# sourmash-bio/sourmash

Measured on AMD Instinct MI355X. Metric: Gbase/s sketched (k=31, scaled=1000), higher is better.
Workload: dtype u64; 1 GPU; C2: sketch synthetic random DNA resident in HBM as ASCII, per GPU 1000 records of 10000000 bases (10000000000 bases, 10000001000 bytes with their separators), k=31 scaled=1000 seed=42; one step = k-mer kernel + radix sort + unique; records_per_gpu=1000, record_len=10000000, bases_per_gpu=10000000000, bytes_per_gpu=10000001000, ksize=31, scaled=1000, unique_hashes_rank0=9998668, unique_hashes_job=9998668, collectives=none (the exchange runs with --full)

## Files before the change

### sourmash_amd/csrc/kmer_core.hpp

```cpp
#pragma once
#include "murmur3.hpp"
#include <utility>

namespace smg {

SMG_HD uint32_t perm_b32(uint32_t hi, uint32_t lo, uint32_t sel) {
#if defined(__HIP_DEVICE_COMPILE__)
    return __builtin_amdgcn_perm(hi, lo, sel);
#else
    const uint64_t v = ((uint64_t)hi << 32) | lo;
    uint32_t r = 0;
    for (int i = 0; i < 4; ++i) {
        const uint32_t s = (sel >> (8 * i)) & 0xff;
        uint32_t b;
        if (s < 8) b = (uint32_t)(v >> (8 * s)) & 0xff;
        else if (s == 0x0c) b = 0;
        else b = 0xff;
        r |= b << (8 * i);
    }
    return r;
#endif
}

SMG_HD uint32_t alignbyte_b32(uint32_t hi, uint32_t lo, uint32_t n) {
#if defined(__HIP_DEVICE_COMPILE__)
    return __builtin_amdgcn_alignbyte(hi, lo, n);
#else
    return (uint32_t)((((uint64_t)hi << 32) | lo) >> (8 * n));
#endif
}

SMG_HD bool any_lane(bool p) {
#if defined(__HIP_DEVICE_COMPILE__)
    return __builtin_amdgcn_ballot_w64(p) != 0ull;
#else
    return p;
#endif
}

SMG_HD uint32_t bitselect(uint32_t mask, uint32_t b, uint32_t c) {
#if defined(__HIP_DEVICE_COMPILE__)
    return __builtin_amdgcn_bitop3_b32(mask, b, c, 0xCA);
#else
    return (mask & b) | (~mask & c);
#endif
}

SMG_HD uint32_t opaque(uint32_t x) {
#if defined(__HIP_DEVICE_COMPILE__)
    asm volatile("" : "+v"(x));
#endif
    return x;
}

SMG_HD uint32_t bswap32(uint32_t x) { return perm_b32(0u, x, 0x00010203u); }

constexpr uint32_t LUT_SELF = 'A' | ('C' << 8) | ('T' << 16) | ((uint32_t)'G' << 24);
constexpr uint32_t LUT_COMP = 'T' | ('G' << 8) | ('A' << 16) | ((uint32_t)'C' << 24);

template <int K, int P>
struct LaneGeom {
    static constexpr int NBYTES = P + K - 1;
    static constexpr int NW = (NBYTES + 3) / 4;
    static constexpr int NWK = (K + 3) / 4;
    static constexpr int NCH = (K + 7) / 8;
    static constexpr uint32_t LAST_MASK = (K % 4) ? ((1u << (8 * (K % 4))) - 1u) : 0xffffffffu;
};

constexpr uint32_t rev_sel(int a) {
    return (uint32_t)(a + 3) | ((uint32_t)(a + 2) << 8) | ((uint32_t)(a + 1) << 16) | ((uint32_t)a << 24);
}
constexpr uint32_t rev_sel_partial(int a, int nb) {
    uint32_t s = 0;
    for (int i = 0; i < 4; ++i) {
        const uint32_t b = (i < nb) ? (uint32_t)(a + nb - 1 - i) : 0x0cu;
        s |= b << (8 * i);
    }
    return s;
}

template <int K, int P, int O>
struct PosOps {
    using G = LaneGeom<K, P>;

    template <int D>
    static SMG_HD uint32_t fwd(const uint32_t* U) {
        constexpr int q = (O >> 2) + D, a = O & 3;
        uint32_t v;
        if constexpr (a == 0) v = U[q];
        else if constexpr (q + 1 < G::NW) v = alignbyte_b32(U[q + 1], U[q], a);
        else v = U[q] >> (8 * a);
        if constexpr (D == G::NWK - 1) v &= G::LAST_MASK;
        return v;
    }

    template <int D>
    static SMG_HD uint32_t rev(const uint32_t* C) {
        constexpr int nb = (K - 4 * D) >= 4 ? 4 : (K - 4 * D);
        constexpr int s = O + K - 4 * D - nb;
        constexpr int q = s >> 2, a = s & 3;
        constexpr uint32_t sel = (nb == 4) ? rev_sel(a) : rev_sel_partial(a, nb);
        if constexpr (q + 1 < G::NW) return perm_b32(C[q + 1], C[q], sel);
        else return perm_b32(0u, C[q], sel);
    }

    template <int CH>
    static SMG_HD uint64_t be_chunk(const uint32_t* W) {
        uint64_t v = (uint64_t)bswap32(W[2 * CH]) << 32;
        if constexpr (2 * CH + 1 < G::NWK) v |= bswap32(W[2 * CH + 1]);
        return v;
    }

    template <int CH>
    static SMG_HD uint64_t be_chunk_opaque(const uint32_t* W) {
        uint64_t v = (uint64_t)bswap32(opaque(W[2 * CH])) << 32;
        if constexpr (2 * CH + 1 < G::NWK) v |= bswap32(opaque(W[2 * CH + 1]));
        return v;
    }

    template <int CH>
    static SMG_HD void tie_break(const uint32_t* F, const uint32_t* R, bool& tie, bool& gt) {
        if constexpr (CH < G::NCH) {
            const uint64_t bf = be_chunk_opaque<CH>(F), br = be_chunk_opaque<CH>(R);
            gt = gt || (tie && bf > br);
            tie = tie && (bf == br);
            tie_break<CH + 1>(F, R, tie, gt);
        }
    }

    template <int... D>
    static SMG_HD void build(const uint32_t* U, const uint32_t* C, uint32_t* F, uint32_t* R,
                             std::integer_sequence<int, D...>) {
        ((F[D] = fwd<D>(U)), ...);
        ((R[D] = rev<D>(C)), ...);
    }

    template <bool PLAIN = false>
    static SMG_HD Mmh3Open hash_open(const uint32_t* U, const uint32_t* C, uint64_t seed) {
        uint32_t F[G::NWK], R[G::NWK];
        build(U, C, F, R, std::make_integer_sequence<int, G::NWK>{});
        const uint64_t bf = be_chunk<0>(F), br = be_chunk<0>(R);
        bool gt = bf > br;
        bool tie = bf == br;
        if (G::NCH > 1 && any_lane(tie)) tie_break<1>(F, R, tie, gt);
        uint32_t W[G::NWK];
        const uint32_t m = gt ? 0xffffffffu : 0u;
#pragma unroll
        for (int d = 0; d < G::NWK; ++d) W[d] = bitselect(m, R[d], F[d]);
        return mmh3_open_words<K, PLAIN>(W, seed);
    }
};

SMG_HD uint32_t nonzero_bytes4(uint32_t x) {
    uint32_t t = x | (x >> 4);
    t |= t >> 2;
    t |= t >> 1;
    t &= 0x01010101u;
    return (t * 0x01020408u) >> 24 & 0xfu;
}

SMG_HD uint32_t early_limit(uint64_t thr) {
    const uint32_t thr_hi = (uint32_t)(thr >> 32);
    return thr_hi >= 0xfffffffdu ? 0xffffffffu : thr_hi + 2u;
}
SMG_HD bool early_may_keep(Mmh3Open open, uint32_t lim) { return (uint32_t)(mmh3_close_hi_sum(open) + 1u) <= lim; }

template <int K, int P, bool EARLY, bool PLAIN, bool STAGED, class Emit, int... O>
SMG_HD void process_window(const uint32_t* raw, const uint32_t* comp, bool dirty, uint64_t seed, uint64_t thr, Emit&& emit,
                           std::integer_sequence<int, O...>) {
    using G = LaneGeom<K, P>;
    const uint32_t lim = early_limit(thr);
    uint32_t Ubuf[STAGED ? 1 : G::NW], Cbuf[STAGED ? 1 : G::NW];
    const uint32_t* U = STAGED ? raw : Ubuf;
    const uint32_t* C = STAGED ? comp : Cbuf;
    uint32_t anybad = 0;
    if constexpr (!STAGED) {
#pragma unroll
        for (int i = 0; i < G::NW; ++i) {
            const uint32_t u = raw[i] & 0xdfdfdfdfu;
            const uint32_t code = (u >> 1) & 0x03030303u;
            Ubuf[i] = u;
            Cbuf[i] = perm_b32(0u, LUT_COMP, code);
            uint32_t bad = perm_b32(0u, LUT_SELF, code) ^ u;
            if (i == G::NW - 1 && (G::NBYTES % 4) != 0)
                bad &= (1u << (8 * (G::NBYTES % 4))) - 1u;
            anybad |= bad;
        }
    }
    uint64_t badlo = 0, badhi = 0, badtop = 0;
    if (!STAGED || dirty) {
        if constexpr (STAGED) {
#pragma unroll
            for (int i = 0; i < G::NW; ++i) {
                const uint32_t u = U[i];
                uint32_t bad = perm_b32(0u, LUT_SELF, (u >> 1) & 0x03030303u) ^ u;
                if (i == G::NW - 1 && (G::NBYTES % 4) != 0)
                    bad &= (1u << (8 * (G::NBYTES % 4))) - 1u;
                anybad |= bad;
            }
        }
        if (anybad != 0) {
#pragma unroll
            for (int i = 0; i < G::NW; ++i) {
                const uint32_t u = U[i];
                const uint32_t code = (u >> 1) & 0x03030303u;
                uint32_t bad = perm_b32(0u, LUT_SELF, code) ^ u;
                if (i == G::NW - 1 && (G::NBYTES % 4) != 0) bad &= (1u << (8 * (G::NBYTES % 4))) - 1u;
                const uint64_t nib = nonzero_bytes4(bad);
                if (4 * i < 64) badlo |= nib << (4 * i);
                else if (4 * i < 128) badhi |= nib << (4 * i - 64);
                else badtop |= nib << (4 * i - 128);
            }
        }
    }
    static_assert(G::NBYTES <= 192 && K <= 128 && P <= 64, "window too long for the 192-bit validity mask");
    (
        [&] {
            const Mmh3Open open = PosOps<K, P, O>::template hash_open<PLAIN>(U, C, seed);
            if constexpr (EARLY) {
                if (!any_lane(early_may_keep(open, lim))) return;
            }
            const uint64_t h = mmh3_close<PLAIN>(open);
            bool ok = (h - 1) < thr;
            if (anybad != 0) {
                uint64_t lo, hi;
                if constexpr (O == 0) { lo = badlo; hi = badhi; }
                else { lo = (badlo >> O) | (badhi << (64 - O)); hi = (badhi >> O) | (badtop << (64 - O)); }
                const uint64_t mlo = K >= 64 ? ~0ull : ((1ull << K) - 1);
                const uint64_t mhi = K >= 128 ? ~0ull : K > 64 ? ((1ull << (K - 64)) - 1) : 0;
                if ((lo & mlo) | (hi & mhi)) ok = false;
            }
            if (ok) emit(O, h);
        }(),
        ...);
}

template <int K, int P, bool EARLY = true, bool PLAIN = false, class Emit>
SMG_HD void process_lane(const uint32_t* raw, uint64_t seed, uint64_t thr, Emit&& emit) {
    process_window<K, P, EARLY, PLAIN, false>(raw, nullptr, false, seed, thr, static_cast<Emit&&>(emit),
                                              std::make_integer_sequence<int, P>{});
}
template <int K, int P, bool EARLY = true, bool PLAIN = false, class Emit>
SMG_HD void process_lane_staged(const uint32_t* U, const uint32_t* C, bool dirty, uint64_t seed, uint64_t thr, Emit&& emit) {
    process_window<K, P, EARLY, PLAIN, true>(U, C, dirty, seed, thr, static_cast<Emit&&>(emit), std::make_integer_sequence<int, P>{});
}


template <int K, int P, int BLOCK>
struct TileGeom {
    using G = LaneGeom<K, P>;
    static constexpr int TILE = BLOCK * P;
    static constexpr int LANE_RD = ((G::NW + 3) / 4) * 4;
    static constexpr int IN_DW = (BLOCK - 1) * (P / 4) + LANE_RD;
    static constexpr int IN_CHUNKS = (IN_DW + 3) / 4;
};

SMG_HD void load_chunk(const uint8_t* seq, uint64_t off, uint64_t len, uint32_t skip, uint32_t* w) {
    w[0] = w[1] = w[2] = w[3] = 0;
    if (off + 16 <= len) {
#if defined(__HIP_DEVICE_COMPILE__)
        const uint4 v = *reinterpret_cast<const uint4*>(seq + off);
        w[0] = v.x; w[1] = v.y; w[2] = v.z; w[3] = v.w;
#else
        for (int b = 0; b < 16; ++b) w[b >> 2] |= (uint32_t)seq[off + b] << (8 * (b & 3));
#endif
    } else if (off < len) {
        for (uint64_t b = off; b < len; ++b) w[(b - off) >> 2] |= (uint32_t)seq[b] << (8 * ((b - off) & 3));
    }
    if (off == 0 && skip) {
        for (uint32_t b = 0; b < skip; ++b) w[b >> 2] &= ~(0xffu << (8 * (b & 3)));
    }
}

SMG_HD uint32_t stage_chunk(uint32_t* w, uint32_t* c) {
    uint32_t anybad = 0;
#pragma unroll
    for (int j = 0; j < 4; ++j) {
        const uint32_t u = w[j] & 0xdfdfdfdfu;
        const uint32_t code = (u >> 1) & 0x03030303u;
        w[j] = u;
        c[j] = perm_b32(0u, LUT_COMP, code);
        anybad |= perm_b32(0u, LUT_SELF, code) ^ u;
    }
    return anybad;
}

SMG_HD void store_chunk(uint32_t* dst, const uint32_t* w) {
#if defined(__HIP_DEVICE_COMPILE__)
    *reinterpret_cast<uint4*>(dst) = make_uint4(w[0], w[1], w[2], w[3]);
#else
    dst[0] = w[0]; dst[1] = w[1]; dst[2] = w[2]; dst[3] = w[3];
#endif
}

template <int IN_CHUNKS, bool STAGED, int BLOCK>
SMG_HD void stage_tile(const uint8_t* seq, uint64_t base, uint64_t len, uint32_t skip, uint32_t* s_in, uint32_t* s_comp,
                       unsigned int* s_dirty) {
#if defined(__HIP_DEVICE_COMPILE__)
    const int first = threadIdx.x, step = BLOCK;
#else
    const int first = 0, step = 1;
#endif
    for (int c = first; c < IN_CHUNKS; c += step) {
        uint32_t w[4];
        load_chunk(seq, base + (uint64_t)c * 16, len, skip, w);
        if constexpr (STAGED) {
            uint32_t cw[4];
            if (stage_chunk(w, cw)) *s_dirty = 1;
            store_chunk(&s_comp[c * 4], cw);
        }
        store_chunk(&s_in[c * 4], w);
    }
}

template <int LANE_RD, int P>
SMG_HD void read_window(const uint32_t* s, int tid, uint32_t* out) {
    static_assert(P % 4 == 0 && LANE_RD % 4 == 0, "lane runs must start dword aligned");
    const uint32_t* p = &s[tid * (P / 4)];
#pragma unroll
    for (int i = 0; i < LANE_RD / 4; ++i) {
#if defined(__HIP_DEVICE_COMPILE__)
        if constexpr ((P / 4) % 4 == 0) {
            const uint4 v = reinterpret_cast<const uint4*>(p)[i];
            out[4 * i] = v.x; out[4 * i + 1] = v.y; out[4 * i + 2] = v.z; out[4 * i + 3] = v.w;
            continue;
        }
#endif
        out[4 * i] = p[4 * i]; out[4 * i + 1] = p[4 * i + 1]; out[4 * i + 2] = p[4 * i + 2]; out[4 * i + 3] = p[4 * i + 3];
    }
}

#if defined(__HIPCC__)
template <int CAP, int BLOCK, int NV = 1>
struct LdsSink {
    uint64_t* s_val[NV];
    unsigned int* s_cnt;
    unsigned long long* s_base;
    uint64_t* out[NV];
    unsigned long long* out_count;
    uint64_t out_cap;

    template <class... V>
    __device__ __forceinline__ void append(V... v) const {
        static_assert(sizeof...(V) == NV, "one value per array");
        const uint64_t e[NV] = {(uint64_t)v...};
        const unsigned int idx = atomicAdd(s_cnt, 1u);
        if (idx < (unsigned)CAP) {
#pragma unroll
            for (int j = 0; j < NV; ++j) s_val[j][idx] = e[j];
        } else {
            const unsigned long long g = atomicAdd(out_count, 1ull);
            if (g < out_cap) {
#pragma unroll
                for (int j = 0; j < NV; ++j) out[j][g] = e[j];
            }
        }
    }
    __device__ __forceinline__ void flush(unsigned int at_least) const {
        const unsigned int cnt = *s_cnt;
        if (cnt < at_least) return;
        const unsigned int n = cnt < (unsigned)CAP ? cnt : (unsigned)CAP;
        if (threadIdx.x == 0) *s_base = atomicAdd(out_count, (unsigned long long)n);
        __syncthreads();
        const unsigned long long b = *s_base;
        for (unsigned int i = threadIdx.x; i < n; i += BLOCK) {
            if (b + i < out_cap) {
#pragma unroll
                for (int j = 0; j < NV; ++j) out[j][b + i] = s_val[j][i];
            }
        }
        __syncthreads();
        if (threadIdx.x == 0) *s_cnt = 0;
    }
};
#endif

}
```

### sourmash_amd/csrc/sketch_kernel.hpp

```cpp
#pragma once
#include <hip/hip_runtime.h>
#include <stdint.h>
#include <utility>
#include "kmer_core.hpp"
#include "tile_launch.hpp"

namespace smg {

constexpr int SK_BLOCK = 256;
constexpr int SK_FAST_MAX_K = 88;
constexpr int SK_OUT_CAP = 2048;

constexpr bool sk_plain_mul(int k, bool dense) {
    if (dense) return k == 1 || k == 5 || k == 8 || k == 25 || k == 28 || k == 81 || k == 82 || k == 84;
    return k == 50 || k == 51;
}
constexpr bool sk_staged(int k) { return k > 11 && k != 18 && k != 20 && k != 30; }

template <int K, int P, bool DENSE>
__global__ __launch_bounds__(SK_BLOCK) void sketch_dna_kernel(
    const uint8_t* __restrict__ seq, uint64_t len, uint64_t seed, uint64_t thr,
    uint64_t* __restrict__ out, unsigned long long* __restrict__ out_count, uint64_t out_cap,
    uint64_t n_tiles, uint32_t skip) {
    using T = TileGeom<K, P, SK_BLOCK>;
    constexpr int TILE = T::TILE, LANE_RD = T::LANE_RD, IN_CHUNKS = T::IN_CHUNKS;
    constexpr bool STAGED = !DENSE && sk_staged(K);

    __shared__ __attribute__((aligned(16))) uint32_t s_in[IN_CHUNKS * 4];
    __shared__ __attribute__((aligned(16))) uint32_t s_comp[STAGED ? IN_CHUNKS * 4 : 4];
    __shared__ unsigned int s_dirty;
    __shared__ uint64_t s_out[SK_OUT_CAP];
    __shared__ unsigned int s_cnt;
    __shared__ unsigned long long s_base;
    const LdsSink<SK_OUT_CAP, SK_BLOCK> sink{{s_out}, &s_cnt, &s_base, {out}, out_count, out_cap};

    const int tid = threadIdx.x;
    if (tid == 0) s_cnt = 0;

    for (uint64_t tile = blockIdx.x; tile < n_tiles; tile += gridDim.x) {
        const uint64_t base = tile * (uint64_t)TILE;
        if constexpr (STAGED) {
            if (tid == 0) s_dirty = 0;
        }
        __syncthreads();
        if constexpr (STAGED) {
            stage_tile<IN_CHUNKS, true, SK_BLOCK>(seq, base, len, skip, s_in, s_comp, &s_dirty);
        } else {
            for (int c = tid; c < IN_CHUNKS; c += SK_BLOCK) {
                const uint64_t off = base + (uint64_t)c * 16;
                uint4 v = make_uint4(0, 0, 0, 0);
                if (off + 16 <= len) {
                    v = *reinterpret_cast<const uint4*>(seq + off);
                } else if (off < len) {
                    uint32_t w[4] = {0, 0, 0, 0};
                    for (uint64_t b = off; b < len; ++b) w[(b - off) >> 2] |= (uint32_t)seq[b] << (8 * ((b - off) & 3));
                    v = make_uint4(w[0], w[1], w[2], w[3]);
                }
                if (off == 0 && skip) {
                    uint32_t w[4] = {v.x, v.y, v.z, v.w};
                    for (uint32_t b = 0; b < skip; ++b) w[b >> 2] &= ~(0xffu << (8 * (b & 3)));
                    v = make_uint4(w[0], w[1], w[2], w[3]);
                }
                *reinterpret_cast<uint4*>(&s_in[c * 4]) = v;
            }
        }
        __syncthreads();
        uint32_t raw[LANE_RD];
        read_window<LANE_RD, P>(s_in, tid, raw);
        auto emit = [&](int o, uint64_t h) {
            if constexpr (DENSE) {
                const uint64_t pos = base + (uint64_t)tid * P + (uint64_t)o - skip;
                if (pos < out_cap) out[pos] = h;
            } else {
                sink.append(h);
            }
        };
        if constexpr (STAGED) {
            static_assert(!STAGED || P == 16, "the staged form reads whole 16-byte groups");
            uint32_t comp[LANE_RD];
            read_window<LANE_RD, P>(s_comp, tid, comp);
            const bool dirty = __builtin_amdgcn_readfirstlane(s_dirty) != 0;
            process_lane_staged<K, P, true, sk_plain_mul(K, false)>(raw, comp, dirty, seed, thr, emit);
        } else {
            process_lane<K, P, !DENSE, sk_plain_mul(K, DENSE)>(raw, seed, thr, emit);
        }
        if constexpr (DENSE) continue;
        __syncthreads();
        sink.flush(SK_OUT_CAP / 2);
    }
    if constexpr (DENSE) return;
    __syncthreads();
    sink.flush(1);
}

typedef hipError_t (*sketch_launch_fn)(const uint8_t*, uint64_t, uint64_t, uint64_t, uint64_t*, unsigned long long*, uint64_t, hipStream_t);
template <bool DENSE>
struct SketchLaunch {
    using fn = sketch_launch_fn;
    static constexpr int KMAX = SK_FAST_MAX_K;
    template <int K>
    static hipError_t launch(const uint8_t* d_seq, uint64_t len, uint64_t seed, uint64_t thr, uint64_t* d_out,
                             unsigned long long* d_count, uint64_t cap, hipStream_t stream) {
        const TileSpan t = align_to_tiles(d_seq, len, (uint64_t)SK_BLOCK * 16);
        if (t.n_tiles == 0) return hipSuccess;
        hipLaunchKernelGGL((sketch_dna_kernel<K, 16, DENSE>), dim3(sk_grid(t.n_tiles)), dim3(SK_BLOCK), 0, stream, t.seq, t.len, seed,
                           thr, d_out, d_count, cap, t.n_tiles, t.skip);
        return hipGetLastError();
    }
};

}
```

### sourmash_amd/csrc/tile_launch.hpp

```cpp
#pragma once
#include <hip/hip_runtime.h>
#include <stdint.h>
#include <utility>

namespace smg {

struct TileSpan {
    const uint8_t* seq;
    uint64_t len;
    uint32_t skip;
    uint64_t n_tiles;
};
inline TileSpan align_to_tiles(const uint8_t* d_seq, uint64_t len, uint64_t tile_positions) {
    const uint32_t skip = (uint32_t)((uintptr_t)d_seq & 15);
    return {d_seq - skip, len + skip, skip, (len + skip + tile_positions - 1) / tile_positions};
}

inline unsigned sk_grid(uint64_t n_tiles) {
    const uint64_t max_blocks = 256ull * 8;
    return (unsigned)(n_tiles < max_blocks ? n_tiles : max_blocks);
}
inline unsigned lds_grid(uint64_t n_tiles, bool lds) {
    uint64_t g = sk_grid(n_tiles);
    if (lds && g > 256 && g > n_tiles / 8) g = n_tiles / 8 > 256 ? n_tiles / 8 : 256;
    return (unsigned)g;
}

template <auto Kernel>
hipError_t allow_dynamic_lds(size_t bytes, size_t most) {
    if (bytes <= 48 * 1024) return hipSuccess;
    static const hipError_t allowed = hipFuncSetAttribute((const void*)Kernel, hipFuncAttributeMaxDynamicSharedMemorySize, (int)most);
    return allowed;
}

constexpr int K_PART = 16;

template <class F, int K0, int... KS>
typename F::fn k_launcher_from(uint32_t k, std::integer_sequence<int, KS...>) {
    static const typename F::fn table[] = {&F::template launch<K0 + KS + 1>...};
    return table[k - K0 - 1];
}
template <class F, int PART>
typename F::fn part_launcher(uint32_t k);
template <class F>
typename F::fn launcher(uint32_t k) {
    static_assert(F::KMAX > 5 * K_PART && F::KMAX <= 6 * K_PART, "six parts");
    switch ((k - 1u) / (uint32_t)K_PART) {
    case 0: return part_launcher<F, 0>(k);
    case 1: return part_launcher<F, 1>(k);
    case 2: return part_launcher<F, 2>(k);
    case 3: return part_launcher<F, 3>(k);
    case 4: return part_launcher<F, 4>(k);
    default: return part_launcher<F, 5>(k);
    }
}
#define SMG_KMER_PART(F, PART)                                                                                                   \
    template <>                                                                                                                  \
    typename F::fn part_launcher<F, PART>(uint32_t k) {                                                                          \
        constexpr int K0 = K_PART * (PART), N = F::KMAX - K0 < K_PART ? F::KMAX - K0 : K_PART;                                   \
        return k_launcher_from<F, K0>(k, std::make_integer_sequence<int, N>());                                                  \
    }

}
```

Measured before the change: 334.1 Gbase/s.

## Stage multiple rounds per tile in LDS and enlarge sketch grid

For staged k>17, each workgroup now loads a tile covering up to three 4096-base windows into LDS with one pair of barriers and one sink flush, then loops over the rounds. This amortises synchronisation, halo reloads and flush overhead across more positions. The LDS output buffer is halved to fit and the grid per CU grows from 8 to 32. Rounds fall back to one when the expected hashes per tile might overflow the smaller sink.

```diff
diff --git a/sourmash_amd/csrc/kmer_core.hpp b/sourmash_amd/csrc/kmer_core.hpp
--- a/sourmash_amd/csrc/kmer_core.hpp
+++ b/sourmash_amd/csrc/kmer_core.hpp
@@ -246,14 +246,23 @@
 }
 
 
-template <int K, int P, int BLOCK>
+template <int K, int P, int BLOCK, int R = 1>
 struct TileGeom {
     using G = LaneGeom<K, P>;
-    static constexpr int TILE = BLOCK * P;
+    static constexpr int WINDOW = BLOCK * P;
+    static constexpr int TILE = R * WINDOW;
     static constexpr int LANE_RD = ((G::NW + 3) / 4) * 4;
-    static constexpr int IN_DW = (BLOCK - 1) * (P / 4) + LANE_RD;
-    static constexpr int IN_CHUNKS = (IN_DW + 3) / 4;
+    static constexpr int chunks(int rounds) { return ((rounds * BLOCK - 1) * (P / 4) + LANE_RD + 3) / 4; }
+    static constexpr int IN_DW = (R * BLOCK - 1) * (P / 4) + LANE_RD;
+    static constexpr int IN_CHUNKS = chunks(R);
 };
+
+SMG_HD uint32_t sk_tile_rounds(uint64_t thr, uint32_t r_max, uint32_t window, uint32_t cap) {
+    if (r_max <= 1) return 1;
+    const uint64_t positions = (uint64_t)r_max * window;
+    const uint64_t expected = (positions * (thr >> 32)) >> 32;
+    return expected + 1 > cap / 4 ? 1u : r_max;
+}
 
 SMG_HD void load_chunk(const uint8_t* seq, uint64_t off, uint64_t len, uint32_t skip, uint32_t* w) {
     w[0] = w[1] = w[2] = w[3] = 0;
@@ -295,13 +304,13 @@
 
 template <int IN_CHUNKS, bool STAGED, int BLOCK>
 SMG_HD void stage_tile(const uint8_t* seq, uint64_t base, uint64_t len, uint32_t skip, uint32_t* s_in, uint32_t* s_comp,
-                       unsigned int* s_dirty) {
+                       unsigned int* s_dirty, int n_chunks = IN_CHUNKS) {
 #if defined(__HIP_DEVICE_COMPILE__)
     const int first = threadIdx.x, step = BLOCK;
 #else
     const int first = 0, step = 1;
 #endif
-    for (int c = first; c < IN_CHUNKS; c += step) {
+    for (int c = first; c < n_chunks; c += step) {
         uint32_t w[4];
         load_chunk(seq, base + (uint64_t)c * 16, len, skip, w);
         if constexpr (STAGED) {
diff --git a/sourmash_amd/csrc/sketch_kernel.hpp b/sourmash_amd/csrc/sketch_kernel.hpp
--- a/sourmash_amd/csrc/sketch_kernel.hpp
+++ b/sourmash_amd/csrc/sketch_kernel.hpp
@@ -16,35 +16,52 @@
     return k == 50 || k == 51;
 }
 constexpr bool sk_staged(int k) { return k > 11 && k != 18 && k != 20 && k != 30; }
+#ifndef SMG_SK_R_MAX
+#define SMG_SK_R_MAX 3
+#endif
+constexpr int SK_R_MAX = SMG_SK_R_MAX;
+static_assert(SK_R_MAX >= 1 && SK_R_MAX <= 3, "four rounds do not fit four workgroups per CU");
+constexpr bool sk_one_round(int k) { return k <= 17; }
+constexpr int sk_rounds_max(int k, bool dense) { return !dense && sk_staged(k) && !sk_one_round(k) ? SK_R_MAX : 1; }
+constexpr int sk_out_cap(int r_max) { return r_max >= 3 ? SK_OUT_CAP / 2 : SK_OUT_CAP; }
+#ifdef SMG_SK_GRID_PER_CU
+constexpr unsigned sk_grid_per_cu(int) { return SMG_SK_GRID_PER_CU; }
+#else
+constexpr unsigned sk_grid_per_cu(int r_max) { return r_max > 1 ? 32 : 8; }
+#endif
 
 template <int K, int P, bool DENSE>
 __global__ __launch_bounds__(SK_BLOCK) void sketch_dna_kernel(
     const uint8_t* __restrict__ seq, uint64_t len, uint64_t seed, uint64_t thr,
     uint64_t* __restrict__ out, unsigned long long* __restrict__ out_count, uint64_t out_cap,
-    uint64_t n_tiles, uint32_t skip) {
-    using T = TileGeom<K, P, SK_BLOCK>;
-    constexpr int TILE = T::TILE, LANE_RD = T::LANE_RD, IN_CHUNKS = T::IN_CHUNKS;
+    uint64_t n_tiles, uint32_t skip, uint32_t rounds) {
+    constexpr int R_MAX = sk_rounds_max(K, DENSE), OUT_CAP = sk_out_cap(R_MAX);
+    using T = TileGeom<K, P, SK_BLOCK, R_MAX>;
+    constexpr int WINDOW = T::WINDOW, LANE_RD = T::LANE_RD, IN_CHUNKS = T::IN_CHUNKS;
     constexpr bool STAGED = !DENSE && sk_staged(K);
+    static_assert(R_MAX == 1 || STAGED, "only the staged form walks several rounds");
+    const uint32_t n_rounds = R_MAX > 1 ? rounds : 1u;
 
     __shared__ __attribute__((aligned(16))) uint32_t s_in[IN_CHUNKS * 4];
     __shared__ __attribute__((aligned(16))) uint32_t s_comp[STAGED ? IN_CHUNKS * 4 : 4];
     __shared__ unsigned int s_dirty;
-    __shared__ uint64_t s_out[SK_OUT_CAP];
+    __shared__ uint64_t s_out[OUT_CAP];
     __shared__ unsigned int s_cnt;
     __shared__ unsigned long long s_base;
-    const LdsSink<SK_OUT_CAP, SK_BLOCK> sink{{s_out}, &s_cnt, &s_base, {out}, out_count, out_cap};
+    const LdsSink<OUT_CAP, SK_BLOCK> sink{{s_out}, &s_cnt, &s_base, {out}, out_count, out_cap};
 
     const int tid = threadIdx.x;
     if (tid == 0) s_cnt = 0;
 
     for (uint64_t tile = blockIdx.x; tile < n_tiles; tile += gridDim.x) {
-        const uint64_t base = tile * (uint64_t)TILE;
+        const uint64_t base = tile * ((uint64_t)n_rounds * WINDOW);
         if constexpr (STAGED) {
             if (tid == 0) s_dirty = 0;
         }
         __syncthreads();
         if constexpr (STAGED) {
-            stage_tile<IN_CHUNKS, true, SK_BLOCK>(seq, base, len, skip, s_in, s_comp, &s_dirty);
+            if constexpr (R_MAX > 1) stage_tile<IN_CHUNKS, true, SK_BLOCK>(seq, base, len, skip, s_in, s_comp, &s_dirty, T::chunks((int)n_rounds));
+            else stage_tile<IN_CHUNKS, true, SK_BLOCK>(seq, base, len, skip, s_in, s_comp, &s_dirty);
         } else {
             for (int c = tid; c < IN_CHUNKS; c += SK_BLOCK) {
                 const uint64_t off = base + (uint64_t)c * 16;
@@ -66,7 +83,7 @@
         }
         __syncthreads();
         uint32_t raw[LANE_RD];
-        read_window<LANE_RD, P>(s_in, tid, raw);
+        if constexpr (R_MAX == 1) read_window<LANE_RD, P>(s_in, tid, raw);
         auto emit = [&](int o, uint64_t h) {
             if constexpr (DENSE) {
                 const uint64_t pos = base + (uint64_t)tid * P + (uint64_t)o - skip;
@@ -78,15 +95,25 @@
         if constexpr (STAGED) {
             static_assert(!STAGED || P == 16, "the staged form reads whole 16-byte groups");
             uint32_t comp[LANE_RD];
-            read_window<LANE_RD, P>(s_comp, tid, comp);
-            const bool dirty = __builtin_amdgcn_readfirstlane(s_dirty) != 0;
-            process_lane_staged<K, P, true, sk_plain_mul(K, false)>(raw, comp, dirty, seed, thr, emit);
+            if constexpr (R_MAX == 1) {
+                read_window<LANE_RD, P>(s_comp, tid, comp);
+                const bool dirty = __builtin_amdgcn_readfirstlane(s_dirty) != 0;
+                process_lane_staged<K, P, true, sk_plain_mul(K, false)>(raw, comp, dirty, seed, thr, emit);
+            } else {
+                const bool dirty = __builtin_amdgcn_readfirstlane(s_dirty) != 0;
+#pragma unroll 1
+                for (uint32_t r = 0; r < n_rounds; ++r) {
+                    read_window<LANE_RD, P>(s_in, tid + (int)r * SK_BLOCK, raw);
+                    read_window<LANE_RD, P>(s_comp, tid + (int)r * SK_BLOCK, comp);
+                    process_lane_staged<K, P, true, sk_plain_mul(K, false)>(raw, comp, dirty, seed, thr, emit);
+                }
+            }
         } else {
             process_lane<K, P, !DENSE, sk_plain_mul(K, DENSE)>(raw, seed, thr, emit);
         }
         if constexpr (DENSE) continue;
         __syncthreads();
-        sink.flush(SK_OUT_CAP / 2);
+        sink.flush(OUT_CAP / 2);
     }
     if constexpr (DENSE) return;
     __syncthreads();
@@ -101,10 +128,12 @@
     template <int K>
     static hipError_t launch(const uint8_t* d_seq, uint64_t len, uint64_t seed, uint64_t thr, uint64_t* d_out,
                              unsigned long long* d_count, uint64_t cap, hipStream_t stream) {
-        const TileSpan t = align_to_tiles(d_seq, len, (uint64_t)SK_BLOCK * 16);
+        constexpr uint32_t WINDOW = (uint32_t)SK_BLOCK * 16, R_MAX = (uint32_t)sk_rounds_max(K, DENSE);
+        const uint32_t rounds = sk_tile_rounds(thr, R_MAX, WINDOW, (uint32_t)sk_out_cap((int)R_MAX));
+        const TileSpan t = align_to_tiles(d_seq, len, (uint64_t)rounds * WINDOW);
         if (t.n_tiles == 0) return hipSuccess;
-        hipLaunchKernelGGL((sketch_dna_kernel<K, 16, DENSE>), dim3(sk_grid(t.n_tiles)), dim3(SK_BLOCK), 0, stream, t.seq, t.len, seed,
-                           thr, d_out, d_count, cap, t.n_tiles, t.skip);
+        hipLaunchKernelGGL((sketch_dna_kernel<K, 16, DENSE>), dim3(sk_grid(t.n_tiles, sk_grid_per_cu((int)R_MAX))), dim3(SK_BLOCK), 0, stream,
+                           t.seq, t.len, seed, thr, d_out, d_count, cap, t.n_tiles, t.skip, rounds);
         return hipGetLastError();
     }
 };
diff --git a/sourmash_amd/csrc/tile_launch.hpp b/sourmash_amd/csrc/tile_launch.hpp
--- a/sourmash_amd/csrc/tile_launch.hpp
+++ b/sourmash_amd/csrc/tile_launch.hpp
@@ -16,8 +16,8 @@
     return {d_seq - skip, len + skip, skip, (len + skip + tile_positions - 1) / tile_positions};
 }
 
-inline unsigned sk_grid(uint64_t n_tiles) {
-    const uint64_t max_blocks = 256ull * 8;
+inline unsigned sk_grid(uint64_t n_tiles, unsigned per_cu = 8) {
+    const uint64_t max_blocks = 256ull * per_cu;
     return (unsigned)(n_tiles < max_blocks ? n_tiles : max_blocks);
 }
 inline unsigned lds_grid(uint64_t n_tiles, bool lds) {
```

New measurement: 363.6 Gbase/s, median of 6. +8.8%, better.
